# sebproell/4C

Measured on AMD Instinct MI355X. Metric: element-evaluations/sec (hex8 linear elasticity, K+r global assembly), higher is better.
Workload: dtype f64; 1 GPU; hex8-linear-100^3-per-gpu; elements_global=1000000, elements_evaluated_per_gpu=1000000, dofs_owned_rank0=3090903, nnz_rank0=245438109

## Files before the change

4c_amd/csrc/fcg_context.cpp:

```cpp
#include <hip/hip_runtime.h>

#include <algorithm>
#include <chrono>
#include <climits>
#include <cstdlib>
#include <cstring>
#include <mutex>
#include <string>
#include <thread>
#include <vector>

#include "fcg_internal.hpp"
#include "fcg_status.hpp"
#include "fcg_shape.hpp"

namespace {

namespace plan = fcg::create;

std::mutex g_err_mutex;
std::string g_create_error;

void set_create_error(const std::string& s)
{
  std::lock_guard<std::mutex> lk(g_err_mutex);
  g_create_error = s;
}

template <class T>
hipError_t upload(T** dst, const T* src, int64_t n, int64_t& bytes)
{
  *dst = nullptr;
  if (n == 0) return hipSuccess;
  hipError_t e = hipMalloc(reinterpret_cast<void**>(dst), sizeof(T) * n);
  if (e != hipSuccess) return e;
  bytes += sizeof(T) * n;
  if (src) return hipMemcpy(*dst, src, sizeof(T) * n, hipMemcpyHostToDevice);
  return hipSuccess;
}

void free_mesh(fcg::DeviceMesh& m)
{
  void* ptrs[] = {m.node_dof_row, m.node_dof_kcol, m.mass_ptr, m.mass_inc, m.mass_tab, m.mass_rho, m.mass_bad, m.stress_tab, m.stress_bad, m.stress_slot, m.explicit_work, m.ele_mat, m.apply_ye, m.apply_dof, m.diag_de, m.diag_dbc, m.gather_dummy, m.multi_ptr, m.rec_row0, m.rec_meta, m.rec_base, m.rec_ele, m.rec_a, m.rec_tmap, m.ele_orig, m.inc_ele, m.inc_a, m.asm_order, m.ele_x,
      m.ele_dof, m.ele_nodes, m.ele_gid, m.node_x, m.node_dof_col, m.inc_of, m.inc_ptr,
      m.rownode_row0, m.inc_pos, m.rowptr, m.scratch, m.err, m.elem_at, m.lat_x, m.lat_dof,
      m.plane_rec, m.reg_rec, m.reg_tile, m.reg_pos,
      m.tables, m.stamps, m.col_lid, m.diag_pos, m.pcg_work, m.krylov_work, m.col_ele, m.ele_ft, m.inc_row0, m.ele_gp,
      m.pen_ptr, m.ele_nb, m.h27_rows, m.h27_rslot0, m.h27_slot};
  for (void* p : ptrs)
    if (p) (void)hipFree(p);
  if (m.err_host) (void)hipHostFree(m.err_host);
  m = fcg::DeviceMesh{};
}

int graph_on_device(const fcg_desc* d, const int32_t* kcol, std::vector<int64_t>& rowptr,
    std::vector<int32_t>& col, std::string& why)
{
  const int npe = d->celltype == FCG_HEX27 ? 27 : 8;
  if (d->n_rows % 3 != 0)
  {
    why = "n_rows must be 3 x owned nodes";
    return FCG_ERR_ARG;
  }
  for (int64_t n = 0; n < d->n_node; ++n)
    if (kcol[n] < 0 || (d->node_dof_row[n] >= 0 && d->node_dof_row[n] % 3 != 0))
    {
      why = "node DOF LIDs must be non-negative and owned rows start at multiples of 3";
      return FCG_ERR_ARG;
    }
// ... 187 lines not shown
  m.sweep_defer = de && de[0] ? de[0] == '1' : d->kinematics == FCG_LINEAR;
  const char* se = std::getenv("FCG_SWEEP_SKIP_EMPTY");
  m.sweep_skip_empty = !(se && se[0] == '0');
  U.up(&m.elem_at, sp.elem_at);
  U.up(&m.lat_x, sp.lat_x);
  U.up(&m.lat_dof, sp.lat_dof);
  U.up(&m.plane_rec, sp.plane_rec);
  const char* rg = std::getenv("FCG_SWEEP_REGULAR");
  const bool regular = !(rg && rg[0] == '0') && d->kinematics == FCG_LINEAR;
  m.layers_total = sp.layers_total;
  m.reg_layers = regular ? sp.reg_layers : 0;
  if (m.reg_layers > 0)
  {
    U.up(&m.reg_rec, sp.reg_rec);
    U.up(&m.reg_tile, sp.reg_tile);
  }
  else
  {
    const std::vector<uint32_t> no_rec(fcg::REG_REC_WORDS, 0u);
    const std::vector<int32_t> no_run(sp.reg_tile.size(), 0);
    U.up(&m.reg_rec, no_rec);
    U.up(&m.reg_tile, no_run);
  }
  int32_t pos32[32] = {};
  std::copy(sp.reg_pos, sp.reg_pos + 27, pos32);
  U.up(&m.reg_pos, pos32, 32);
  std::vector<double> tab(8 * 8 * 3 * 2 + 8 + 24);
  double xi[81], w[27], xn[81];
  fcg::gauss_rule(fcg::kHex8, xi, w);
  fcg::node_param_coords(fcg::kHex8, xn);
  for (int g = 0; g < 8; ++g) fcg::shape_deriv(fcg::kHex8, &xi[3 * g], &tab[24 * g]);
  for (int g = 0; g < 8; ++g) fcg::shape_deriv(fcg::kHex8, &xn[3 * g], &tab[192 + 24 * g]);
  for (int g = 0; g < 8; ++g) tab[384 + g] = w[g];
  for (int k = 0; k < 24; ++k) tab[392 + k] = xi[k];
  U.up(&m.tables, tab);
  const char* ck = std::getenv("FCG_SWEEP_CHECKED");
  if (U.he == hipSuccess) U.chk(fcg::sweep_geometry_pass(m, ck && ck[0] == '1', U.ctx->stream));
}

void upload_colored(Uploader& U, const fcg_desc* d, const plan::Incidences& I, const plan::ColorHost& cp)
{
  fcg::DeviceMesh& m = U.ctx->mesh;
  m.path = FCG_PATH_COLORED;
  U.up(&m.inc_of, I.inc_of);
  U.up(&m.inc_pos, I.inc_pos);
  U.up(&m.inc_row0, I.inc_row0);
  m.h27_pencil = d->material == FCG_MAT_STVK;
  if (m.h27_pencil)
  {
    fcg::upload_h27_tables();
    U.up(&m.col_ele, cp.pen_ele.data(), d->n_ele);
    U.up(&m.pen_ptr, cp.pen_ptr);
    U.up(&m.ele_nb, cp.nb.data(), d->n_ele);
    for (int c = 0; c < 5; ++c) m.pen_color[c] = cp.pen_color[c];
  }
  else
  {
    U.up(&m.col_ele, cp.col_ele.data(), d->n_ele);
    U.up(&m.ele_ft, cp.ft.data(), d->n_ele);
    for (int c = 0; c < 9; ++c) m.color_ptr[c] = cp.color_ptr[c];
// ... 503 lines not shown
  return FCG_OK;
}

int fcg_get_timing(const fcg_ctx* ctx, double* ms_element, double* ms_assemble)
{
  if (!ctx) return FCG_ERR_ARG;
  read_timing(const_cast<fcg_ctx*>(ctx)->timing);
  if (ms_element) *ms_element = ctx->timing.ms_element;
  if (ms_assemble) *ms_assemble = ctx->timing.ms_assemble;
  return 2;
}

int fcg_get_diagnostics(const fcg_ctx* ctx, uint64_t* out, int n)
{
  if (!ctx || !out || n < 0) return FCG_ERR_ARG;
  const fcg::DeviceMesh& m = ctx->mesh;
  unsigned long long v[16] = {};
  if (m.stamps && hipMemcpy(v, m.stamps, sizeof(v), hipMemcpyDeviceToHost) != hipSuccess)
    return fcg_device_error();
  v[15] = m.path != FCG_PATH_STRUCTURED ? FCG_SWEEP_KERNEL_NA
                                        : (m.sweep_checked ? FCG_SWEEP_KERNEL_CHECKED : FCG_SWEEP_KERNEL_UNCHECKED);
  v[13] = m.path == FCG_PATH_STRUCTURED && !m.sweep_checked ? uint64_t(m.reg_layers) : 0;
  v[14] = m.path == FCG_PATH_STRUCTURED ? uint64_t(m.layers_total) : 0;
  v[12] = m.path != FCG_PATH_STRUCTURED ? FCG_SWEEP_ROWS_NA
                                        : (m.sweep_defer ? FCG_SWEEP_ROWS_DEFERRED : FCG_SWEEP_ROWS_DIRECT);
  for (int i = 0; i < n && i < 16; ++i) out[i] = v[i];
  return m.stamps ? 16 : 0;
}

int fcg_get_create_phases(const fcg_ctx* ctx, double* out, int n)
{
  if (!ctx || (!out && n > 0)) return FCG_ERR_ARG;
  for (int i = 0; i < n && i < 8; ++i) out[i] = ctx->create_phase_s[i];
  return 8;
}

int fcg_get_info(const fcg_ctx* ctx, fcg_info* info)
{
  if (!ctx || !info) return FCG_ERR_ARG;
  const fcg::DeviceMesh& m = ctx->mesh;
  info->n_ele = m.n_ele;
  info->n_node = m.n_node;
  info->n_rows = m.n_rows;
  info->n_cols = m.n_cols;
  info->nnz = m.nnz;
  info->n_incidences = m.n_inc;
// ... 138 lines not shown
```

4c_amd/csrc/fcg_create_plan.cpp:

```cpp
#include "fcg_create_plan.hpp"

#include <array>
#include <climits>
#include <cstdlib>
#include <cstring>
#include <map>
#include <mutex>

#include "fcg_shape.hpp"

namespace fcg {
namespace create {

const int kOff8[8][3] = {{0, 0, 0}, {1, 0, 0}, {1, 1, 0}, {0, 1, 0}, {0, 0, 1}, {1, 0, 1}, {1, 1, 1},
    {0, 1, 1}};

uint64_t morton_key(const double* x, const double* lo, const double* hi)
{
  uint64_t key = 0;
  uint32_t q[3];
  for (int k = 0; k < 3; ++k)
  {
    const double ext = hi[k] - lo[k];
    const double t = ext > 0 ? (x[k] - lo[k]) / ext : 0.0;
// ... 389 lines not shown
  P.tiles_x = (P.n[0] + 3) / 4;
  P.tiles_y = (P.n[1] + 3) / 4;
  const int64_t txy = int64_t(P.tiles_x) * P.tiles_y;
  const char* wenv = std::getenv("FCG_SWEEP_WGS_PER_CU");
  const int wpc = wenv ? std::max(1, std::atoi(wenv)) : 2;
  const char* tenv = std::getenv("FCG_SWEEP_TOTLAG_WGS_PER_CU");
  const int tpc = tenv ? std::max(1, std::atoi(tenv)) : 1;
  const int64_t slots = int64_t(std::max(1, cus)) * (d->kinematics == FCG_TOTLAG ? tpc : wpc);
  int64_t nseg = 1;
  double best = 0.0;
  for (int64_t k = 1; k <= std::min<int64_t>(P.n[2], 64); ++k)
  {
    const int64_t segk = (P.n[2] + k - 1) / k;
    const int64_t wgs = txy * ((P.n[2] + segk - 1) / segk);
    const double cost = double((wgs + slots - 1) / slots) * double(segk + 1);
    if (k == 1 || cost < best)
    {
      best = cost;
      nseg = k;
    }
  }
  P.seg = int32_t((P.n[2] + nseg - 1) / nseg);
  P.tiles_z = (P.n[2] + P.seg - 1) / P.seg;
  P.lat_x.assign(3 * NXn * NYn * NZn, 0.0);
  P.lat_dof.assign(NXn * NYn * NZn, -1);
  for (int64_t nd = 0; nd < d->n_node; ++nd)
  {
    if (npos[nd] < 0) continue;
    for (int k = 0; k < 3; ++k) P.lat_x[3 * npos[nd] + k] = d->node_x[3 * nd + k];
    P.lat_dof[npos[nd]] = d->node_dof_col[nd];
  }
  const int64_t W = fcg::PLANE_REC_WORDS;
  P.plane_rec.assign(int64_t(P.tiles_y) * P.tiles_x * P.n[2] * W, 0u);
  parallel_for(int64_t(P.tiles_y) * P.tiles_x * P.n[2], [&](int64_t idx) {
    const int64_t k = idx % P.n[2];
    const int64_t t = idx / P.n[2];
    const int64_t tx = t % P.tiles_x, ty = t / P.tiles_x;
    uint32_t* rec = P.plane_rec.data() + idx * W;
    uint16_t* np = reinterpret_cast<uint16_t*>(rec + 64);
    for (int c = 0; c < 16; ++c)
    {
      const int64_t i = 4 * tx + c % 4, jj = 4 * ty + c / 4;
      int32_t r = -1;
      if (i < P.n[0] && jj < P.n[1]) r = P.rownode_at[(k * P.n[1] + jj) * P.n[0] + i];
      if (r < 0)
      {
        rec[c] = 0xFFFFFFFFu;
        for (int q = 0; q < 27; ++q) np[27 * c + q] = 0xFFFF;
        continue;
      }
      const int64_t base = d->rowptr[row0[r]];
      rec[c] = uint32_t(row0[r]);
      rec[16 + c] = uint32_t(d->rowptr[row0[r] + 1] - base);
      rec[32 + 2 * c] = uint32_t(uint64_t(base) & 0xFFFFFFFFu);
      rec[32 + 2 * c + 1] = uint32_t(uint64_t(base) >> 32);
      for (int q = 0; q < 27; ++q) np[27 * c + q] = P.nbr_pos[r * 27 + q];
    }
  });
  classify_regular_tiles(P);
  return true;
}

void classify_regular_tiles(StructHost& P)
{
  const int64_t W = fcg::PLANE_REC_WORDS, NK = P.n[2];
  const int64_t ntile = int64_t(P.tiles_y) * P.tiles_x;
  P.reg_rec.assign(ntile * NK * REG_REC_WORDS, 0u);
  P.reg_tile.assign(2 * ntile, 0);
  std::fill(P.reg_pos, P.reg_pos + 27, 0);
  P.reg_layers = 0;
  P.layers_total = 0;
  std::map<std::array<uint16_t, 27>, int64_t> seen;
  const int64_t nrn = int64_t(P.nbr_pos.size()) / 27;
  for (int64_t r = 0; r < nrn; ++r)
  {
    std::array<uint16_t, 27> a;
    bool full = true;
    for (int t = 0; t < 27; ++t)
    {
      a[t] = P.nbr_pos[r * 27 + t];
      full = full && a[t] != 0xFFFF;
    }
// ... 643 lines not shown
```

4c_amd/csrc/fcg_create_plan.hpp:

```cpp
#pragma once

#include <algorithm>
#include <atomic>
#include <cstdint>
#include <string>
#include <thread>
#include <vector>

#include "fourc_gpu.h"

namespace fcg {

constexpr int PLANE_REC_WORDS = 288;
constexpr int REG_REC_WORDS = 16;

namespace create {

template <class F>
void parallel_for(int64_t n, F f)
{
  unsigned nt = std::max(1u, std::min(16u, std::thread::hardware_concurrency()));
  if (n < 4096) nt = 1;
  std::vector<std::thread> th;
  std::atomic<int64_t> next{0};
  const int64_t chunk = 1024;
  auto body = [&]() {
    for (;;)
    {
      const int64_t s = next.fetch_add(chunk);
      if (s >= n) break;
      const int64_t e = std::min(n, s + chunk);
      for (int64_t i = s; i < e; ++i) f(i);
    }
  };
  for (unsigned t = 1; t < nt; ++t) th.emplace_back(body);
  body();
  for (auto& t : th) t.join();
// ... 16 lines not shown
  bool triple_rows = true;
  std::vector<int64_t> diag;
  bool rowcol = false;
  bool square_local = false;
  bool owned_cols_first = false;
  int64_t nrn() const { return int64_t(rownodes.size()); }
};
int build_node_rows(const fcg_desc* d, NodeRows& N, std::string& why);
void build_operator_support(const fcg_desc* d, NodeRows& N);

struct StructHost {
  int32_t lo[3] = {0, 0, 0}, n[3] = {0, 0, 0};
  int32_t elo[3] = {0, 0, 0}, en[3] = {0, 0, 0};
  int32_t tiles_x = 0, tiles_y = 0, tiles_z = 0, seg = 0;
  std::vector<int32_t> elem_at, rownode_at;
  std::vector<uint16_t> nbr_pos;
  std::vector<double> lat_x;
  std::vector<int32_t> lat_dof;
  std::vector<uint32_t> plane_rec;
  std::vector<uint32_t> reg_rec;
  std::vector<int32_t> reg_tile;
  int32_t reg_pos[27] = {};
  int64_t reg_layers = 0, layers_total = 0;
};
void classify_regular_tiles(StructHost& P);
bool detect_lattice_hex8(const fcg_desc* d, std::vector<int32_t>& ijk, std::vector<int32_t>& canon,
    std::string& why);
bool build_structured_plan(const fcg_desc* d, const std::vector<int32_t>& rownodes,
    const std::vector<int32_t>& row0, const int32_t* kcol, int cus, StructHost& P, std::string& why);

struct ColorHost {
  std::vector<int32_t> col_ele;
  std::vector<uint8_t> ft;
  int64_t color_ptr[9] = {0, 0, 0, 0, 0, 0, 0, 0, 0};
  std::vector<int32_t> pen_ele;
  std::vector<int64_t> pen_ptr;
  int64_t pen_color[5] = {0, 0, 0, 0, 0};
  std::vector<uint32_t> nb;
};
bool build_colored_plan(const fcg_desc* d, ColorHost& P, std::string& why);

struct PathChoice {
  bool structured = false, colored = false, gather = false;
  StructHost sp;
  ColorHost cp;
  int path() const
  {
// ... 54 lines not shown
```

4c_amd/csrc/fcg_internal.hpp:

```cpp
#pragma once

#include <hip/hip_runtime.h>

#include <cstdint>
#include <string>
#include <vector>

#include "fcg_create_plan.hpp"
#include "fourc_gpu.h"

namespace fcg {

#ifndef FCG_REC27
#define FCG_REC27 256
#endif
constexpr int64_t record_doubles(int npe) { return npe == 27 ? int64_t(FCG_REC27) : 9 * int64_t(npe) + 3; }

struct DeviceMesh {
  int celltype = 0, kinem = 0, npe = 8;
  int64_t n_ele = 0, n_node = 0, n_rows = 0, n_cols = 0, nnz = 0;
  int64_t n_rownodes = 0, n_inc = 0;
  double lambda = 0, mu = 0, cdiag = 0;
  int material = FCG_MAT_STVK;
  double nh_c = 0, nh_beta = 0;
// ... 49 lines not shown
  int64_t h27_nslab = 0, h27_slab = 0, h27_ring = 0;
  int h27_el_grid = 512;
  std::vector<int64_t> h27_asm_ptr;
  int32_t* h27_rows = nullptr;
  int32_t* h27_rslot0 = nullptr;
  int32_t* h27_slot = nullptr;

  int path = FCG_PATH_GENERAL;
  int32_t tiles_x = 0, tiles_y = 0, tiles_z = 0, seg_planes = 0;
  int32_t I0 = 0, J0 = 0, K0 = 0, NI = 0, NJ = 0, NK = 0;
  int32_t EX0 = 0, EY0 = 0, EZ0 = 0, EX = 0, EY = 0, EZ = 0;
  bool sweep_defer = false;
  bool sweep_skip_empty = true;
  int32_t geom_code = 0, geom_ele = INT32_MAX;
  bool geom_neg = false, sweep_checked = true;
  int32_t* elem_at = nullptr;
  double* lat_x = nullptr;
  int32_t* lat_dof = nullptr;
  uint32_t* plane_rec = nullptr;
  uint32_t* reg_rec = nullptr;
  int32_t* reg_tile = nullptr;
  int32_t* reg_pos = nullptr;
  int64_t reg_layers = 0, layers_total = 0;
  double* tables = nullptr;
  unsigned long long* stamps = nullptr;

  int32_t* col_lid = nullptr;
  int64_t* diag_pos = nullptr;
  bool square_local = false;
  bool owned_cols_first = false;
  bool triple_rows = true;
  double* pcg_work = nullptr;
  int64_t pcg_n = 0;

  int32_t* node_dof_row = nullptr;
  int32_t* node_dof_kcol = nullptr;
  int64_t* mass_ptr = nullptr;
  int64_t* mass_inc = nullptr;
  double* mass_tab = nullptr;
  double* mass_rho = nullptr;
  int32_t* mass_bad = nullptr;

  double* stress_tab = nullptr;
  double* stress_xinv = nullptr;
  int32_t* stress_bad = nullptr;
  int32_t* stress_slot = nullptr;
// ... 106 lines not shown
```

4c_amd/csrc/fcg_sweep.hip:

```cpp
#include <hip/hip_runtime.h>

#include <type_traits>

#include "fcg_hex8_element.hpp"
#include "fcg_internal.hpp"
#include "fcg_visit_table.h"

namespace fcg {

namespace {

constexpr int TX = 4, TY = 4;
constexpr int EXN = TX + 1, EYN = TY + 1;
constexpr int NSLOT = EXN * EYN;
constexpr int NXN = TX + 2;
constexpr int NNODE = NXN * (TY + 2);
constexpr int PR_ROW0 = 0, PR_LEN = 16, PR_BASE = 32, PR_NPOS = 64;
__device__ constexpr int nx_sw(int p, int slot) { return (p + 4 * (slot & 1)) & 7; }
__device__ constexpr int nx2i(int d, int p, int slot, int n)
{
  return (((d * 4 + p) * NSLOT + slot) * 8 + (n ^ nx_sw(p, slot))) * 2;
}

__device__ constexpr int node_ox(int n) { return ((n & 3) == 1 || (n & 3) == 2) ? 1 : 0; }
// ... 3 lines not shown
struct SweepArgs {
  const double* u_col;
  const double* lat_x;
  const int32_t* lat_dof;
  const int32_t* elem_at;
  const uint32_t* plane_rec;
  const uint32_t* reg_rec;
  const int32_t* reg_tile;
  const int32_t* reg_pos;
  const double* tables;
  double* K;
  double* fint;
  int32_t* err;
  unsigned long long* stamps;
  StVK mat;
  const double* v_col;
  const double* T_col;
  const double* Ngp;
  double* Kst;
  double* Kts;
  double* Ktt;
  double* fT;
  double tsi_m, tsi_T0, tsi_k, tsi_kts;
  int32_t tiles_x, tiles_y, seg_planes;
  int32_t I0, J0, K0, NI, NJ, NK;
  int32_t EX0, EY0, EZ0, EX, EY, EZ;
  int32_t skip_empty;
};

template <bool TSI>
constexpr int node_comps() { return TSI ? 10 : 6; }

#ifndef FCG_GP_STRIDE
#define FCG_GP_STRIDE 18
#endif
#ifndef FCG_TG_STRIDE
#define FCG_TG_STRIDE 4
#endif

template <int KIN, bool TSI, bool TH = false, bool DEFER = false>
struct SweepShared {
  alignas(16) double nx[3 * 4 * NSLOT * 8 * 2];
  alignas(16) double gp[KIN ? 8 : 1][KIN ? NSLOT : 1][KIN ? FCG_GP_STRIDE : 16];
  alignas(16) double tg[TSI ? 8 : 1][TSI ? NSLOT : 1][TSI ? FCG_TG_STRIDE : 4];
  double node[3][NNODE][node_comps<TSI>()];
  uint32_t prec[3][PLANE_REC_WORDS];
  double gxi[8][4];
  double Ng[TSI ? 8 : 1][8];
  alignas(16) double NgT[TSI ? 8 : 1][10];
  double w8[8];
// ... 393 lines not shown
  if (A.stamps && tid == 0)                                                                        \
  {                                                                                                \
    const unsigned long long now = __builtin_amdgcn_s_memtime();                                  \
    st_acc[i] += now - st_last;                                                                    \
    st_last = now;                                                                                 \
  }

template <int KIN, bool WANT_K, bool OVERWRITE, int MODE, bool CHECKED = true>
#ifndef FCG_SWEEP_WGS
#define FCG_SWEEP_WGS 2
#endif
__global__ __launch_bounds__(256, KIN ? 1 : FCG_SWEEP_WGS) void sweep_h8_kernel(SweepArgs A)
{
  constexpr bool TSI = MODE == 1 || MODE == 2, TH = MODE == 2, DEFER = MODE == 3, GEOM = MODE == 4;
  static_assert(!GEOM || (KIN == 0 && !WANT_K && CHECKED), "the geometry pass is one instantiation");
  static_assert(CHECKED || !TSI, "the TSI passes keep the checks");
  static_assert(!TSI || (KIN == 0 && WANT_K), "TSI is geometrically linear, full tangent");
  static_assert(!DEFER || WANT_K, "deferred blocks are K blocks");
  __shared__ SweepShared<KIN, TSI, TH, DEFER> sh;
  constexpr int NACC = TH ? 8 : ((KIN || TSI) ? 16 : 9);
  constexpr int NC = node_comps<TSI>();
  constexpr int NLD = (NNODE * NC + 255) / 256;
  constexpr int NF = TSI ? 4 : 3;
  const int tid = threadIdx.x;
  unsigned long long st_acc[3] = {0, 0, 0};
  unsigned long long st_last = A.stamps ? __builtin_amdgcn_s_memtime() : 0ull;
  const int tile = blockIdx.x;
  const int tx = tile % A.tiles_x;
  const int ty = (tile / A.tiles_x) % A.tiles_y;
  const int tz = tile / (A.tiles_x * A.tiles_y);
  const int i0 = A.I0 + TX * tx, j0 = A.J0 + TY * ty;
  const int kz0 = A.K0 + A.seg_planes * tz;
  const int kz1 = min(kz0 + A.seg_planes, A.K0 + A.NK);
  const uint32_t* prec_tile = A.plane_rec + (int64_t(ty) * A.tiles_x + tx) * A.NK * PLANE_REC_WORDS;
  const int64_t LX = A.EX + 1, LY = A.EY + 1;
  constexpr bool REGK = (MODE == 0 || MODE == 3) && KIN == 0 && !CHECKED;
  int rlo = 0, rhi = 0;
  const uint32_t* creg_tile = nullptr;
  if constexpr (REGK)
  {
    const int64_t txy = int64_t(ty) * A.tiles_x + tx;
    rlo = max(A.K0 + A.reg_tile[2 * txy], kz0);
    rhi = min(A.K0 + A.reg_tile[2 * txy + 1], kz1) - 1;
    creg_tile = A.reg_rec + txy * A.NK * REG_REC_WORDS;
  }
  auto reg_layer = [&](int L) -> bool { return REGK && L >= rlo && L < rhi; };
  auto reg_plane = [&](int p) -> bool { return REGK && p > rlo && p < rhi; };

  if (tid < 24) sh.gxi[tid / 3][tid % 3] = A.tables[392 + tid];
  if (tid < 8) sh.w8[tid] = A.tables[384 + tid];
  if (TSI && tid < 64)
  {
    (&sh.Ng[0][0])[tid] = A.Ngp[tid];
    sh.NgT[TSI ? (tid & 7) : 0][tid >> 3] = A.Ngp[tid];
  }

  const int s = tid >> 3, g = tid & 7;
  const bool a_lane = s < NSLOT;
  const int sx = s % EXN, sy = s / EXN;
  const int ex = i0 - 1 + sx, ey = j0 - 1 + sy;
  const bool exy_in = a_lane && ex >= A.EX0 && ex < A.EX0 + A.EX && ey >= A.EY0 && ey < A.EY0 + A.EY;
  auto load_elem = [&](int lz) -> int {
    if (reg_layer(lz)) return a_lane ? 0 : -1;
    if (!exy_in || lz < A.EZ0 || lz >= A.EZ0 + A.EZ) return -1;
    return A.elem_at[(int64_t(lz - A.EZ0) * A.EY + (ey - A.EY0)) * A.EX + (ex - A.EX0)];
  };
  bool n_lane[NLD], nxy_in[NLD];
  int ncol[NLD], ncomp[NLD];
  int64_t nlat_xy[NLD];
#pragma unroll
  for (int j = 0; j < NLD; ++j)
  {
    const int v = tid + 256 * j;
    n_lane[j] = v < NNODE * NC;
    ncol[j] = v / NC;
    ncomp[j] = v - NC * (v / NC);
    const int ni = i0 - 1 + ncol[j] % NXN, nj = j0 - 1 + ncol[j] / NXN;
    nxy_in[j] = n_lane[j] && ni >= A.EX0 && ni <= A.EX0 + A.EX && nj >= A.EY0 && nj <= A.EY0 + A.EY;
    nlat_xy[j] = nxy_in[j] ? int64_t(nj - A.EY0) * LX + (ni - A.EX0) : 0;
  }
  auto node_li = [&](int j, int P) -> int64_t { return int64_t(P - A.EZ0) * LX * LY + nlat_xy[j]; };
  auto node_in = [&](int j, int P) -> bool { return nxy_in[j] && P >= A.EZ0 && P <= A.EZ0 + A.EZ; };
  auto load_dof = [&](int j, int P) -> int32_t {
    if (GEOM || !node_in(j, P) || ncomp[j] < 3) return -1;
    return A.lat_dof[node_li(j, P)];
  };
  auto load_val = [&](int j, int P, int32_t dof) -> double {
    const int cp = ncomp[j];
    const bool has = node_in(j, P) && (cp < 3 || dof >= 0);
    const double* src = A.lat_x + (3 * node_li(j, P) + cp);
    if (cp >= 3) src = A.u_col + (dof + cp - 3);
    if (TSI && cp >= 6) src = A.v_col + (dof + cp - 6);
    if (TSI && cp >= 9) src = A.T_col + dof / 3;
    return has ? *src : 0.0;
  };
  auto load_node = [&](int j, int P) -> double { return load_val(j, P, load_dof(j, P)); };
  auto load_rec = [&](int p, uint32_t* w) {
    const bool in = p >= kz0 && p < kz1;
    const uint32_t* src = prec_tile + int64_t(in ? p - A.K0 : 0) * PLANE_REC_WORDS;
    const bool cp = reg_plane(p);
    if (cp) src = creg_tile + int64_t(p - A.K0) * REG_REC_WORDS;
#pragma unroll
    for (int k = 0; k < 2; ++k)
    {
      const int v = tid + 256 * k;
      if (v < PLANE_REC_WORDS) w[k] = (in && (!cp || v < 12)) ? src[v] : (v < PR_LEN ? 0xFFFFFFFFu : 0u);
    }
  };
  auto store_rec = [&](int p, const uint32_t* w) {
    const bool cp = reg_plane(p);
#pragma unroll
    for (int k = 0; k < 2; ++k)
    {
      const int v = tid + 256 * k;
      const int at = cp ? (v < 4 ? PR_ROW0 + 4 * v : PR_BASE + 8 * (((v - 4) >> 1) & 3) + (v & 1)) : v;
      if (v < PLANE_REC_WORDS && (!cp || v < 12)) sh.prec[ring(p)][at] = w[k];
    }
  };

  const int c = tid >> 4, k = tid & 15;
  const int cx = c % TX, cy = c / TX;
  const uint32_t vis0 = kVisit[k][0], vis1 = kVisit[k][1];
  int32_t rp_a = 0, rp_b = 0, rp_s = 0;
  if constexpr (REGK && WANT_K)
  {
    rp_a = A.reg_pos[(vis0 >> 16) & 31] + 243 * cx;
    rp_b = A.reg_pos[(vis1 >> 16) & 31] + 243 * cx;
    rp_s = A.reg_pos[(vis1 >> 11) & 31] + 243 * cx;
  }

  constexpr bool SKIPE = KIN == 0 && !TSI && !GEOM;
  const bool skip_e = SKIPE && A.skip_empty != 0;
  const int L0 = (skip_e && kz0 - 1 < A.EZ0) ? kz0 : kz0 - 1;
#pragma unroll
  for (int j = 0; j < NLD; ++j)
    if (n_lane[j])
    {
      sh.node[ring(L0)][ncol[j]][ncomp[j]] = load_node(j, L0);
      sh.node[ring(L0 + 1)][ncol[j]][ncomp[j]] = load_node(j, L0 + 1);
    }
  {
    uint32_t w[2];
    load_rec(L0, w);
    store_rec(L0, w);
    load_rec(L0 + 1, w);
    store_rec(L0 + 1, w);
  }
  int32_t dof_nxt[NLD];
#pragma unroll
  for (int j = 0; j < NLD; ++j) dof_nxt[j] = n_lane[j] ? load_dof(j, L0 + 2) : -1;
  int e_cur = load_elem(L0);
  for (int v = tid; v < int(sizeof(sh.hold) / sizeof(double)); v += 256) (&sh.hold[0][0][0])[v] = 0.0;
  if constexpr (DEFER)
// ... 462 lines not shown
#ifdef FCG_PROBE_TH_NORMW
            if (OVERWRITE)
#else
            if (OVERWRITE && !TH)
#endif
              A.fint[row0 + d] = fp[d] + f[d];
            else
              A.fint[row0 + d] += fp[d] + f[d];
          }
          if (TSI)
          {
            if (OVERWRITE)
              A.fT[row0 / 3] = fp[NF - 1] + f[NF - 1];
            else
              A.fT[row0 / 3] += fp[NF - 1] + f[NF - 1];
          }
        }
      }
    }
    e_cur = e_nxt;
    __syncthreads();
    FCG_STAMP(1);
  }
  if (A.stamps && tid == 0)
  {
    for (int i = 0; i < 3; ++i) atomicAdd(&A.stamps[i], st_acc[i]);
    atomicAdd(&A.stamps[5], 1ull);
  }
}

}

namespace {
SweepArgs sweep_args(const DeviceMesh& m, const double* d_u_col, double* d_K, double* d_fint)
{
  SweepArgs a{};
  a.u_col = d_u_col;
  a.lat_x = m.lat_x;
  a.lat_dof = m.lat_dof;
  a.elem_at = m.elem_at;
  a.plane_rec = m.plane_rec;
  a.reg_rec = m.reg_rec;
  a.reg_tile = m.reg_tile;
  a.reg_pos = m.reg_pos;
  a.tables = m.tables;
  a.K = d_K;
  a.fint = d_fint;
  a.err = m.err;
  a.stamps = m.stamps;
  a.mat = StVK{m.lambda, m.mu, m.cdiag};
  a.tiles_x = m.tiles_x;
  a.tiles_y = m.tiles_y;
  a.seg_planes = m.seg_planes;
  a.I0 = m.I0; a.J0 = m.J0; a.K0 = m.K0; a.NI = m.NI; a.NJ = m.NJ; a.NK = m.NK;
  a.EX0 = m.EX0; a.EY0 = m.EY0; a.EZ0 = m.EZ0; a.EX = m.EX; a.EY = m.EY; a.EZ = m.EZ;
  a.skip_empty = m.sweep_skip_empty ? 1 : 0;
  return a;
}
}

#define FCG_SWEEP_C(KIN, CHECKED)                                                                  \
  if (want_k && m.sweep_defer && overwrite)                                                        \
    hipLaunchKernelGGL((sweep_h8_kernel<KIN, true, true, 3, CHECKED>), grid, block, 0, stream, a);  \
  else if (want_k && m.sweep_defer)                                                                \
    hipLaunchKernelGGL((sweep_h8_kernel<KIN, true, false, 3, CHECKED>), grid, block, 0, stream, a); \
  else if (want_k && overwrite)                                                                    \
    hipLaunchKernelGGL((sweep_h8_kernel<KIN, true, true, 0, CHECKED>), grid, block, 0, stream, a);  \
  else if (want_k)                                                                                 \
    hipLaunchKernelGGL((sweep_h8_kernel<KIN, true, false, 0, CHECKED>), grid, block, 0, stream, a); \
  else if (overwrite)                                                                              \
    hipLaunchKernelGGL((sweep_h8_kernel<KIN, false, true, 0, CHECKED>), grid, block, 0, stream, a); \
  else                                                                                             \
    hipLaunchKernelGGL((sweep_h8_kernel<KIN, false, false, 0, CHECKED>), grid, block, 0, stream, a);
#define FCG_SWEEP(KIN)                                                                             \
  if (m.sweep_checked)                                                                             \
  {                                                                                                \
    FCG_SWEEP_C(KIN, true)                                                                         \
  }                                                                                                \
  else                                                                                             \
  {                                                                                                \
    FCG_SWEEP_C(KIN, false)                                                                        \
  }

hipError_t launch_sweep_h8_totlag(const DeviceMesh& m, const double* d_u_col, bool want_k,
    bool overwrite, double* d_K, double* d_fint, hipStream_t stream);

#ifdef FCG_SWEEP_TOTLAG_TU
hipError_t launch_sweep_h8_totlag(const DeviceMesh& m, const double* d_u_col, bool want_k,
    bool overwrite, double* d_K, double* d_fint, hipStream_t stream)
{
  const int64_t ntiles = int64_t(m.tiles_x) * m.tiles_y * m.tiles_z;
  if (ntiles == 0) return hipSuccess;
  const SweepArgs a = sweep_args(m, d_u_col, d_K, d_fint);
  const dim3 grid{static_cast<unsigned>(ntiles), 1, 1};
  const dim3 block{256, 1, 1};
  FCG_SWEEP(1)
  return hipGetLastError();
}
#else
hipError_t launch_sweep_h8(const DeviceMesh& m, const double* d_u_col, bool want_k,
    bool overwrite, double* d_K, double* d_fint, hipStream_t stream)
{
  if (m.kinem != 0) return launch_sweep_h8_totlag(m, d_u_col, want_k, overwrite, d_K, d_fint, stream);
  const int64_t ntiles = int64_t(m.tiles_x) * m.tiles_y * m.tiles_z;
  if (ntiles == 0) return hipSuccess;
  const SweepArgs a = sweep_args(m, d_u_col, d_K, d_fint);
  const dim3 grid{static_cast<unsigned>(ntiles), 1, 1};
  const dim3 block{256, 1, 1};
  FCG_SWEEP(0)
  return hipGetLastError();
}

hipError_t sweep_geometry_pass(DeviceMesh& m, bool force_checked, hipStream_t stream)
{
  m.geom_code = 0;
  m.geom_ele = INT32_MAX;
  m.geom_neg = false;
  m.sweep_checked = true;
  const int64_t ntiles = int64_t(m.tiles_x) * m.tiles_y * m.tiles_z;
  if (ntiles > 0)
  {
    int32_t* d_out = nullptr;
    int32_t out[3] = {0, INT32_MAX, 0};
    hipError_t he = hipMalloc(reinterpret_cast<void**>(&d_out), sizeof(out));
    if (he != hipSuccess) return he;
    he = hipMemcpyAsync(d_out, out, sizeof(out), hipMemcpyHostToDevice, stream);
    if (he == hipSuccess)
    {
      SweepArgs a = sweep_args(m, nullptr, nullptr, nullptr);
      a.err = d_out;
      a.stamps = nullptr;
      const dim3 grid{static_cast<unsigned>(ntiles), 1, 1};
      const dim3 block{256, 1, 1};
      hipLaunchKernelGGL((sweep_h8_kernel<0, false, false, 4>), grid, block, 0, stream, a);
      he = hipGetLastError();
    }
    if (he == hipSuccess) he = hipMemcpyAsync(out, d_out, sizeof(out), hipMemcpyDeviceToHost, stream);
    if (he == hipSuccess) he = hipStreamSynchronize(stream);
    (void)hipFree(d_out);
    if (he != hipSuccess) return he;
    m.geom_code = out[0];
    m.geom_ele = out[1];
    m.geom_neg = out[2] != 0;
  }
  m.sweep_checked = force_checked || m.geom_code != 0 || m.geom_neg;
  return hipSuccess;
}

hipError_t launch_sweep_h8_tsi(const DeviceMesh& m, const double* d_u_col, bool overwrite,
    double* d_K, double* d_fint, const SweepTsi& t, hipStream_t stream)
{
  const int64_t ntiles = int64_t(m.tiles_x) * m.tiles_y * m.tiles_z;
  if (ntiles == 0) return hipSuccess;
  SweepArgs a = sweep_args(m, d_u_col, d_K, d_fint);
  a.v_col = t.v_col;
  a.T_col = t.T_col;
  a.Ngp = t.Ngp;
  a.Kst = t.Kst;
  a.Kts = t.Kts;
  a.Ktt = t.Ktt;
  a.fT = t.fT;
  a.tsi_m = t.m;
  a.tsi_T0 = t.T0;
  a.tsi_k = t.conduct;
  a.tsi_kts = t.kts;
  const dim3 grid{static_cast<unsigned>(ntiles), 1, 1};
  const dim3 block{256, 1, 1};
  if (!t.split)
  {
    if (overwrite)
      hipLaunchKernelGGL((sweep_h8_kernel<0, true, true, 1>), grid, block, 0, stream, a);
    else
      hipLaunchKernelGGL((sweep_h8_kernel<0, true, false, 1>), grid, block, 0, stream, a);
    return hipGetLastError();
  }
  if (overwrite)
  {
    hipLaunchKernelGGL((sweep_h8_kernel<0, true, true, 0>), grid, block, 0, stream, a);
    hipLaunchKernelGGL((sweep_h8_kernel<0, true, true, 2>), grid, block, 0, stream, a);
  }
  else
  {
    hipLaunchKernelGGL((sweep_h8_kernel<0, true, false, 0>), grid, block, 0, stream, a);
    hipLaunchKernelGGL((sweep_h8_kernel<0, true, false, 2>), grid, block, 0, stream, a);
  }
  return hipGetLastError();
}
#endif
#undef FCG_SWEEP
// ... 4 lines not shown
```

4c_amd/fcg.py:

```python

import ctypes
import os

import numpy as np

PKG_DIR = os.path.dirname(os.path.abspath(__file__))
LIB_PATH = os.path.join(PKG_DIR, "lib", "libfourc_gpu.so")
if os.environ.get("FCG_LIB"):
    LIB_PATH = os.path.join(PKG_DIR, "lib", "libfourc_gpu_%s.so" % os.environ["FCG_LIB"])

HEX8, HEX27 = 0, 1
LINEAR, TOTLAG = 0, 1
CALC_NLNSTIFF, CALC_INTERNALFORCE = 0, 1
ACCUMULATE, OVERWRITE = 0, 1
PATH_AUTO, PATH_GENERAL, PATH_STRUCTURED, PATH_COLORED, PATH_GATHER = 0, 1, 2, 3, 4
MAT_STVK, MAT_ELASTHYPER_COUPNEOHOOKE = 0, 1
TSI_STRUCT_FORCE, TSI_STIFFTEMP, TSI_THERMO_FINTCOND, TSI_COUPLTANG = 1, 2, 4, 8
TSI_ALL = 15
STRESS_NONE, STRESS_PK2, STRESS_CAUCHY = 0, 1, 2
STRAIN_NONE, STRAIN_GL, STRAIN_EA = 0, 1, 2
ABI_VERSION = 2

FCG_OK, FCG_ERR_NODAL_DETJ, FCG_ERR_SINGULAR, FCG_ERR_ARG, FCG_ERR_DEVICE = 0, 1, 2, 3, 4
STATUS = {0: "FCG_OK", 1: "FCG_ERR_NODAL_DETJ", 2: "FCG_ERR_SINGULAR", 3: "FCG_ERR_ARG",
# ... 926 lines not shown
        buf = (ctypes.c_uint64 * 16)()
        n = lib().fcg_get_diagnostics(self._h, buf, 16)
        return list(buf) if n > 0 else None

    SWEEP_KERNELS = ("not applicable", "checked", "unchecked")

    def sweep_kernel(self):
        buf = (ctypes.c_uint64 * 16)()
        lib().fcg_get_diagnostics(self._h, buf, 16)
        return self.SWEEP_KERNELS[int(buf[15])]

    SWEEP_ROWS = ("not applicable", "direct", "deferred")

    def sweep_rows(self):
        buf = (ctypes.c_uint64 * 16)()
        lib().fcg_get_diagnostics(self._h, buf, 16)
        return self.SWEEP_ROWS[int(buf[12])]

    def sweep_regular_layers(self):
        buf = (ctypes.c_uint64 * 16)()
        lib().fcg_get_diagnostics(self._h, buf, 16)
        return int(buf[13]), int(buf[14])

    CREATE_PHASES = ("checks", "graph_device", "node_rows", "lattice_plans", "incidences",
                     "incidence_positions", "device_plans", "total")

    def create_phases(self):
        buf = (ctypes.c_double * 8)()
        lib().fcg_get_create_phases(self._h, buf, 8)
        return dict(zip(self.CREATE_PHASES, list(buf)))

    def timing(self):
        a, b = ctypes.c_double(), ctypes.c_double()
        lib().fcg_get_timing(self._h, ctypes.byref(a), ctypes.byref(b))
        return a.value, b.value


def gmres_options(restart=None, max_iter=None, rtol=None, precond=None):
    opt = FcgGmresOptions()
    lib().fcg_gmres_default_options(ctypes.byref(opt))
    for k, v in (("restart", restart), ("max_iter", max_iter), ("precond", precond)):
        if v is not None:
            setattr(opt, k, int(v))
    if rtol is not None:
        opt.rtol = float(rtol)
    return opt
# ... 230 lines not shown
```

Measured before the change: 1.188 billion element-evaluations/s.

## Drive sweep kernel from per-block chain records of tile z-segments

Replaces the fixed tile-by-z-segment grid mapping with a host-built table of chains. Each chain lists up to four (tile, kz0, kz1) pieces, and each block loops over the pieces in its record. The default chains match the previous segmentation, so default behaviour should be equivalent. Env vars FCG_SWEEP_CHAINS can select balanced multi-piece or stacked chains, meant to cut tail imbalance and the repeated warm-up plane per segment. The per-block constant setup moves out of the piece loop, and the kernel gains a loop with kernarg re-reads, which may raise register pressure.

```diff
diff --git a/4c_amd/csrc/fcg_context.cpp b/4c_amd/csrc/fcg_context.cpp
--- a/4c_amd/csrc/fcg_context.cpp
+++ b/4c_amd/csrc/fcg_context.cpp
@@ -44,7 +44,7 @@
   void* ptrs[] = {m.node_dof_row, m.node_dof_kcol, m.mass_ptr, m.mass_inc, m.mass_tab, m.mass_rho, m.mass_bad, m.stress_tab, m.stress_bad, m.stress_slot, m.explicit_work, m.ele_mat, m.apply_ye, m.apply_dof, m.diag_de, m.diag_dbc, m.gather_dummy, m.multi_ptr, m.rec_row0, m.rec_meta, m.rec_base, m.rec_ele, m.rec_a, m.rec_tmap, m.ele_orig, m.inc_ele, m.inc_a, m.asm_order, m.ele_x,
       m.ele_dof, m.ele_nodes, m.ele_gid, m.node_x, m.node_dof_col, m.inc_of, m.inc_ptr,
       m.rownode_row0, m.inc_pos, m.rowptr, m.scratch, m.err, m.elem_at, m.lat_x, m.lat_dof,
-      m.plane_rec, m.reg_rec, m.reg_tile, m.reg_pos,
+      m.plane_rec, m.reg_rec, m.reg_tile, m.reg_pos, m.chains, m.seg_chains == m.chains ? nullptr : m.seg_chains,
       m.tables, m.stamps, m.col_lid, m.diag_pos, m.pcg_work, m.krylov_work, m.col_ele, m.ele_ft, m.inc_row0, m.ele_gp,
       m.pen_ptr, m.ele_nb, m.h27_rows, m.h27_rslot0, m.h27_slot};
   for (void* p : ptrs)
@@ -278,6 +278,15 @@
     U.up(&m.reg_rec, no_rec);
     U.up(&m.reg_tile, no_run);
   }
+  U.up(&m.chains, sp.chains.rec);
+  m.n_chains = sp.chains.n;
+  m.chain_longest = sp.chains.longest;
+  m.chain_shortest = sp.chains.shortest;
+  if (sp.chains.rec == sp.seg_chains.rec)
+    m.seg_chains = m.chains;
+  else
+    U.up(&m.seg_chains, sp.seg_chains.rec);
+  m.n_seg_chains = sp.seg_chains.n;
   int32_t pos32[32] = {};
   std::copy(sp.reg_pos, sp.reg_pos + 27, pos32);
   U.up(&m.reg_pos, pos32, 32);
@@ -292,6 +301,14 @@
   U.up(&m.tables, tab);
   const char* ck = std::getenv("FCG_SWEEP_CHECKED");
   if (U.he == hipSuccess) U.chk(fcg::sweep_geometry_pass(m, ck && ck[0] == '1', U.ctx->stream));
+  if (m.sweep_checked && m.chains != m.seg_chains)
+  {
+    (void)hipFree(m.chains);
+    m.chains = m.seg_chains;
+    m.n_chains = sp.seg_chains.n;
+    m.chain_longest = sp.seg_chains.longest;
+    m.chain_shortest = sp.seg_chains.shortest;
+  }
 }
 
 void upload_colored(Uploader& U, const fcg_desc* d, const plan::Incidences& I, const plan::ColorHost& cp)
@@ -841,6 +858,12 @@
                                         : (m.sweep_checked ? FCG_SWEEP_KERNEL_CHECKED : FCG_SWEEP_KERNEL_UNCHECKED);
   v[13] = m.path == FCG_PATH_STRUCTURED && !m.sweep_checked ? uint64_t(m.reg_layers) : 0;
   v[14] = m.path == FCG_PATH_STRUCTURED ? uint64_t(m.layers_total) : 0;
+  if (m.path == FCG_PATH_STRUCTURED)
+  {
+    v[9] = uint64_t(m.n_chains);
+    v[10] = uint64_t(m.chain_longest);
+    v[11] = uint64_t(m.chain_shortest);
+  }
   v[12] = m.path != FCG_PATH_STRUCTURED ? FCG_SWEEP_ROWS_NA
                                         : (m.sweep_defer ? FCG_SWEEP_ROWS_DEFERRED : FCG_SWEEP_ROWS_DIRECT);
   for (int i = 0; i < n && i < 16; ++i) out[i] = v[i];
diff --git a/4c_amd/csrc/fcg_create_plan.cpp b/4c_amd/csrc/fcg_create_plan.cpp
--- a/4c_amd/csrc/fcg_create_plan.cpp
+++ b/4c_amd/csrc/fcg_create_plan.cpp
@@ -435,6 +435,18 @@
   }
   P.seg = int32_t((P.n[2] + nseg - 1) / nseg);
   P.tiles_z = (P.n[2] + P.seg - 1) / P.seg;
+  const char* senv = std::getenv("FCG_SWEEP_SKIP_EMPTY");
+  P.skip_bottom = d->kinematics == FCG_LINEAR && !(senv && senv[0] == '0') && P.lo[2] - 1 < P.elo[2];
+  build_sweep_chains(P, 0, P.seg_chains);
+  P.chains = P.seg_chains;
+  const char* cenv = std::getenv("FCG_SWEEP_CHAINS");
+  if (d->kinematics == FCG_LINEAR)
+  {
+    if (cenv && cenv[0] == 's')
+      build_stacked_chains(P, std::max(1, std::atoi(cenv + 1)), P.chains);
+    else if (cenv && cenv[0])
+      build_sweep_chains(P, std::max(0, std::atoi(cenv)), P.chains);
+  }
   P.lat_x.assign(3 * NXn * NYn * NZn, 0.0);
   P.lat_dof.assign(NXn * NYn * NZn, -1);
   for (int64_t nd = 0; nd < d->n_node; ++nd)
@@ -471,6 +483,128 @@
     }
   });
   classify_regular_tiles(P);
+  return true;
+}
+
+void build_sweep_chains(const StructHost& P, int64_t want, StructHost::Chains& C)
+{
+  const int64_t NK = P.n[2], T = int64_t(P.tiles_x) * P.tiles_y;
+  C = StructHost::Chains{};
+  if (NK <= 0 || T <= 0) return;
+  auto warm = [&](int64_t k) -> int64_t { return (k == 0 && P.skip_bottom) ? 0 : 1; };
+  std::vector<int32_t> cost;
+  auto finish = [&]() {
+    C.n = int32_t(cost.size());
+    C.longest = *std::max_element(cost.begin(), cost.end());
+    C.shortest = *std::min_element(cost.begin(), cost.end());
+  };
+  if (want <= 0)
+  {
+    for (int64_t tz = 0; tz < P.tiles_z; ++tz)
+      for (int64_t t = 0; t < T; ++t)
+      {
+        const int64_t kz0 = int64_t(P.seg) * tz, kz1 = std::min<int64_t>(kz0 + P.seg, NK);
+        int32_t r[SWEEP_CHAIN_WORDS] = {int32_t(t), int32_t(kz0), int32_t(kz1), 0};
+        C.rec.insert(C.rec.end(), r, r + SWEEP_CHAIN_WORDS);
+        cost.push_back(int32_t(kz1 - kz0 + warm(kz0)));
+      }
+    finish();
+    return;
+  }
+  int64_t n = std::min<int64_t>(want, T * NK);
+  for (;;)
+  {
+    C.rec.clear();
+    cost.clear();
+    int64_t t = 0, k = 0;
+    bool capped = false;
+    while (t < T)
+    {
+      const int64_t m = std::max<int64_t>(1, n - int64_t(cost.size()));
+      const int64_t left = (T - t) * NK - k + warm(k) + (T - t - 1) * warm(0) + (m - 1);
+      const int64_t target = std::max<int64_t>((left + m - 1) / m, warm(k) + 1);
+      int32_t r[SWEEP_CHAIN_WORDS] = {};
+      int64_t c = 0;
+      int np = 0;
+      while (t < T && np < SWEEP_CHAIN_PIECES && target - c > warm(k))
+      {
+        const int64_t take = std::min(NK - k, target - c - warm(k));
+        r[4 * np] = int32_t(t);
+        r[4 * np + 1] = int32_t(k);
+        r[4 * np + 2] = int32_t(k + take);
+        c += take + warm(k);
+        ++np;
+        k += take;
+        if (k == NK)
+        {
+          k = 0;
+          ++t;
+        }
+      }
+      capped = capped || (t < T && target - c > warm(k));
+      C.rec.insert(C.rec.end(), r, r + SWEEP_CHAIN_WORDS);
+      cost.push_back(int32_t(c));
+    }
+    if (!capped) break;
+    n = std::max<int64_t>(n + 1, int64_t(cost.size()));
+  }
+  finish();
+}
+
+bool build_stacked_chains(const StructHost& P, int64_t slots, StructHost::Chains& C)
+{
+  const int64_t NK = P.n[2], T = int64_t(P.tiles_x) * P.tiles_y;
+  C = P.seg_chains;
+  if (NK <= 0 || T <= 0 || slots <= 0) return false;
+  const int64_t q = T / slots, R = T % slots;
+  int64_t seg2 = NK, tz2 = 1, rounds2 = R > 0 ? 1 : 0;
+  if (R > 0)
+  {
+    double best = 0.0;
+    for (int64_t k = 1; k <= std::min<int64_t>(NK, 64); ++k)
+    {
+      const int64_t segk = (NK + k - 1) / k, tzk = (NK + segk - 1) / segk;
+      const int64_t rounds = (R * tzk + slots - 1) / slots;
+      const double cost = double(rounds) * double(segk + 1);
+      if (k == 1 || cost < best)
+      {
+        best = cost;
+        seg2 = segk;
+        tz2 = tzk;
+        rounds2 = rounds;
+      }
+    }
+  }
+  if (q == 0 || q + rounds2 > SWEEP_CHAIN_PIECES) return false;
+  auto warm = [&](int64_t k) -> int64_t { return (k == 0 && P.skip_bottom) ? 0 : 1; };
+  C = StructHost::Chains{};
+  std::vector<int32_t> cost;
+  for (int64_t j = 0; j < slots; ++j)
+  {
+    int32_t r[SWEEP_CHAIN_WORDS] = {};
+    int np = 0;
+    int64_t c = 0;
+    auto piece = [&](int64_t t, int64_t k0, int64_t k1) {
+      r[4 * np] = int32_t(t);
+      r[4 * np + 1] = int32_t(k0);
+      r[4 * np + 2] = int32_t(k1);
+      c += k1 - k0 + warm(k0);
+      ++np;
+    };
+    for (int64_t w = 0; w < q; ++w) piece(w * slots + j, 0, NK);
+    for (int64_t w = 0; w < rounds2; ++w)
+    {
+      const int64_t p = w * slots + j;
+      if (p >= R * tz2) break;
+      const int64_t tz = p / R;
+      piece(q * slots + p % R, tz * seg2, std::min((tz + 1) * seg2, NK));
+    }
+    C.rec.insert(C.rec.end(), r, r + SWEEP_CHAIN_WORDS);
+    cost.push_back(int32_t(c));
+  }
+  C.n = int32_t(cost.size());
+  C.longest = *std::max_element(cost.begin(), cost.end());
+  C.shortest = *std::min_element(cost.begin(), cost.end());
   return true;
 }
 
diff --git a/4c_amd/csrc/fcg_create_plan.hpp b/4c_amd/csrc/fcg_create_plan.hpp
--- a/4c_amd/csrc/fcg_create_plan.hpp
+++ b/4c_amd/csrc/fcg_create_plan.hpp
@@ -13,6 +13,8 @@
 
 constexpr int PLANE_REC_WORDS = 288;
 constexpr int REG_REC_WORDS = 16;
+constexpr int SWEEP_CHAIN_PIECES = 4;
+constexpr int SWEEP_CHAIN_WORDS = 4 * SWEEP_CHAIN_PIECES;
 
 namespace create {
 
@@ -75,7 +77,15 @@
   std::vector<int32_t> reg_tile;
   int32_t reg_pos[27] = {};
   int64_t reg_layers = 0, layers_total = 0;
+  struct Chains {
+    std::vector<int32_t> rec;
+    int32_t n = 0, longest = 0, shortest = 0;
+  };
+  Chains chains, seg_chains;
+  bool skip_bottom = false;
 };
+void build_sweep_chains(const StructHost& P, int64_t want, StructHost::Chains& C);
+bool build_stacked_chains(const StructHost& P, int64_t slots, StructHost::Chains& C);
 void classify_regular_tiles(StructHost& P);
 bool detect_lattice_hex8(const fcg_desc* d, std::vector<int32_t>& ijk, std::vector<int32_t>& canon,
     std::string& why);
diff --git a/4c_amd/csrc/fcg_internal.hpp b/4c_amd/csrc/fcg_internal.hpp
--- a/4c_amd/csrc/fcg_internal.hpp
+++ b/4c_amd/csrc/fcg_internal.hpp
@@ -95,6 +95,9 @@
   int32_t* reg_tile = nullptr;
   int32_t* reg_pos = nullptr;
   int64_t reg_layers = 0, layers_total = 0;
+  int32_t* chains = nullptr;
+  int32_t* seg_chains = nullptr;
+  int32_t n_chains = 0, n_seg_chains = 0, chain_longest = 0, chain_shortest = 0;
   double* tables = nullptr;
   unsigned long long* stamps = nullptr;
 
diff --git a/4c_amd/csrc/fcg_sweep.hip b/4c_amd/csrc/fcg_sweep.hip
--- a/4c_amd/csrc/fcg_sweep.hip
+++ b/4c_amd/csrc/fcg_sweep.hip
@@ -49,10 +49,11 @@
   double* Ktt;
   double* fT;
   double tsi_m, tsi_T0, tsi_k, tsi_kts;
-  int32_t tiles_x, tiles_y, seg_planes;
+  int32_t tiles_x, tiles_y;
   int32_t I0, J0, K0, NI, NJ, NK;
   int32_t EX0, EY0, EZ0, EX, EY, EZ;
   int32_t skip_empty;
+  const int32_t* chains;
 };
 
 template <bool TSI>
@@ -492,44 +493,68 @@
   constexpr int NC = node_comps<TSI>();
   constexpr int NLD = (NNODE * NC + 255) / 256;
   constexpr int NF = TSI ? 4 : 3;
-  const int tid = threadIdx.x;
+  const int tid0 = threadIdx.x;
   unsigned long long st_acc[3] = {0, 0, 0};
   unsigned long long st_last = A.stamps ? __builtin_amdgcn_s_memtime() : 0ull;
-  const int tile = blockIdx.x;
-  const int tx = tile % A.tiles_x;
-  const int ty = (tile / A.tiles_x) % A.tiles_y;
-  const int tz = tile / (A.tiles_x * A.tiles_y);
-  const int i0 = A.I0 + TX * tx, j0 = A.J0 + TY * ty;
-  const int kz0 = A.K0 + A.seg_planes * tz;
-  const int kz1 = min(kz0 + A.seg_planes, A.K0 + A.NK);
-  const uint32_t* prec_tile = A.plane_rec + (int64_t(ty) * A.tiles_x + tx) * A.NK * PLANE_REC_WORDS;
   const int64_t LX = A.EX + 1, LY = A.EY + 1;
+  if (tid0 < 24) sh.gxi[tid0 / 3][tid0 % 3] = A.tables[392 + tid0];
+  if (tid0 < 8) sh.w8[tid0] = A.tables[384 + tid0];
+  if (TSI && tid0 < 64)
+  {
+    (&sh.Ng[0][0])[tid0] = A.Ngp[tid0];
+    sh.NgT[TSI ? (tid0 & 7) : 0][tid0 >> 3] = A.Ngp[tid0];
+  }
   constexpr bool REGK = (MODE == 0 || MODE == 3) && KIN == 0 && !CHECKED;
+  const int c = tid0 >> 4, k = tid0 & 15;
+  const int cx = c % TX, cy = c / TX;
+  const uint32_t vis0 = kVisit[k][0], vis1 = kVisit[k][1];
+  int32_t rp_a = 0, rp_b = 0, rp_s = 0;
+  if constexpr (REGK && WANT_K)
+  {
+    rp_a = A.reg_pos[(vis0 >> 16) & 31] + 243 * cx;
+    rp_b = A.reg_pos[(vis1 >> 16) & 31] + 243 * cx;
+    rp_s = A.reg_pos[(vis1 >> 11) & 31] + 243 * cx;
+  }
+
+  constexpr int kPieces = (KIN == 0 && !TSI && !GEOM && !CHECKED) ? SWEEP_CHAIN_PIECES : 1;
+  typedef const SweepArgs __attribute__((address_space(4)))* ArgSegment;
+  ArgSegment Ap = (ArgSegment)__builtin_amdgcn_kernarg_segment_ptr();
+#pragma nounroll
+  for (int piece = 0; piece < kPieces; ++piece)
+  {
+  if constexpr (kPieces > 1) __asm__ volatile("" : "+s"(Ap));
+  int tid_piece = tid0;
+  if constexpr (kPieces > 1) __asm__ volatile("" : "+v"(tid_piece));
+  const int tid = tid_piece;
+#define FCG_COLD(f) (kPieces > 1 ? Ap->f : A.f)
+  const int32_t* chain = FCG_COLD(chains) + (int64_t(blockIdx.x) * SWEEP_CHAIN_WORDS + 4 * piece);
+  const int tile = __builtin_amdgcn_readfirstlane(chain[0]);
+  const int kz0 = FCG_COLD(K0) + __builtin_amdgcn_readfirstlane(chain[1]);
+  const int kz1 = FCG_COLD(K0) + __builtin_amdgcn_readfirstlane(chain[2]);
+  if (kz0 >= kz1) break;
+  const int tx = tile % FCG_COLD(tiles_x);
+  const int ty = tile / FCG_COLD(tiles_x);
+  const int i0 = FCG_COLD(I0) + TX * tx, j0 = FCG_COLD(J0) + TY * ty;
+  const uint32_t* prec_tile = FCG_COLD(plane_rec) + int64_t(tile) * FCG_COLD(NK) * PLANE_REC_WORDS;
+  const int cEX0 = FCG_COLD(EX0), cEY0 = FCG_COLD(EY0), cEX = FCG_COLD(EX), cEY = FCG_COLD(EY);
   int rlo = 0, rhi = 0;
   const uint32_t* creg_tile = nullptr;
   if constexpr (REGK)
   {
-    const int64_t txy = int64_t(ty) * A.tiles_x + tx;
-    rlo = max(A.K0 + A.reg_tile[2 * txy], kz0);
-    rhi = min(A.K0 + A.reg_tile[2 * txy + 1], kz1) - 1;
-    creg_tile = A.reg_rec + txy * A.NK * REG_REC_WORDS;
+    const int32_t* run = FCG_COLD(reg_tile) + 2 * tile;
+    rlo = max(FCG_COLD(K0) + __builtin_amdgcn_readfirstlane(run[0]), kz0);
+    rhi = min(FCG_COLD(K0) + __builtin_amdgcn_readfirstlane(run[1]), kz1) - 1;
+    creg_tile = FCG_COLD(reg_rec) + int64_t(tile) * FCG_COLD(NK) * REG_REC_WORDS;
+#undef FCG_COLD
   }
   auto reg_layer = [&](int L) -> bool { return REGK && L >= rlo && L < rhi; };
   auto reg_plane = [&](int p) -> bool { return REGK && p > rlo && p < rhi; };
-
-  if (tid < 24) sh.gxi[tid / 3][tid % 3] = A.tables[392 + tid];
-  if (tid < 8) sh.w8[tid] = A.tables[384 + tid];
-  if (TSI && tid < 64)
-  {
-    (&sh.Ng[0][0])[tid] = A.Ngp[tid];
-    sh.NgT[TSI ? (tid & 7) : 0][tid >> 3] = A.Ngp[tid];
-  }
 
   const int s = tid >> 3, g = tid & 7;
   const bool a_lane = s < NSLOT;
   const int sx = s % EXN, sy = s / EXN;
   const int ex = i0 - 1 + sx, ey = j0 - 1 + sy;
-  const bool exy_in = a_lane && ex >= A.EX0 && ex < A.EX0 + A.EX && ey >= A.EY0 && ey < A.EY0 + A.EY;
+  const bool exy_in = a_lane && ex >= cEX0 && ex < cEX0 + cEX && ey >= cEY0 && ey < cEY0 + cEY;
   auto load_elem = [&](int lz) -> int {
     if (reg_layer(lz)) return a_lane ? 0 : -1;
     if (!exy_in || lz < A.EZ0 || lz >= A.EZ0 + A.EZ) return -1;
@@ -546,8 +571,8 @@
     ncol[j] = v / NC;
     ncomp[j] = v - NC * (v / NC);
     const int ni = i0 - 1 + ncol[j] % NXN, nj = j0 - 1 + ncol[j] / NXN;
-    nxy_in[j] = n_lane[j] && ni >= A.EX0 && ni <= A.EX0 + A.EX && nj >= A.EY0 && nj <= A.EY0 + A.EY;
-    nlat_xy[j] = nxy_in[j] ? int64_t(nj - A.EY0) * LX + (ni - A.EX0) : 0;
+    nxy_in[j] = n_lane[j] && ni >= cEX0 && ni <= cEX0 + cEX && nj >= cEY0 && nj <= cEY0 + cEY;
+    nlat_xy[j] = nxy_in[j] ? int64_t(nj - cEY0) * (int64_t(cEX) + 1) + (ni - cEX0) : 0;
   }
   auto node_li = [&](int j, int P) -> int64_t { return int64_t(P - A.EZ0) * LX * LY + nlat_xy[j]; };
   auto node_in = [&](int j, int P) -> bool { return nxy_in[j] && P >= A.EZ0 && P <= A.EZ0 + A.EZ; };
@@ -588,17 +613,6 @@
     }
   };
 
-  const int c = tid >> 4, k = tid & 15;
-  const int cx = c % TX, cy = c / TX;
-  const uint32_t vis0 = kVisit[k][0], vis1 = kVisit[k][1];
-  int32_t rp_a = 0, rp_b = 0, rp_s = 0;
-  if constexpr (REGK && WANT_K)
-  {
-    rp_a = A.reg_pos[(vis0 >> 16) & 31] + 243 * cx;
-    rp_b = A.reg_pos[(vis1 >> 16) & 31] + 243 * cx;
-    rp_s = A.reg_pos[(vis1 >> 11) & 31] + 243 * cx;
-  }
-
   constexpr bool SKIPE = KIN == 0 && !TSI && !GEOM;
   const bool skip_e = SKIPE && A.skip_empty != 0;
   const int L0 = (skip_e && kz0 - 1 < A.EZ0) ? kz0 : kz0 - 1;
@@ -1107,7 +1121,8 @@
     __syncthreads();
     FCG_STAMP(1);
   }
-  if (A.stamps && tid == 0)
+  }
+  if (A.stamps && tid0 == 0)
   {
     for (int i = 0; i < 3; ++i) atomicAdd(&A.stamps[i], st_acc[i]);
     atomicAdd(&A.stamps[5], 1ull);
@@ -1136,7 +1151,7 @@
   a.mat = StVK{m.lambda, m.mu, m.cdiag};
   a.tiles_x = m.tiles_x;
   a.tiles_y = m.tiles_y;
-  a.seg_planes = m.seg_planes;
+  a.chains = m.chains;
   a.I0 = m.I0; a.J0 = m.J0; a.K0 = m.K0; a.NI = m.NI; a.NJ = m.NJ; a.NK = m.NK;
   a.EX0 = m.EX0; a.EY0 = m.EY0; a.EZ0 = m.EZ0; a.EX = m.EX; a.EY = m.EY; a.EZ = m.EZ;
   a.skip_empty = m.sweep_skip_empty ? 1 : 0;
@@ -1174,10 +1189,9 @@
 hipError_t launch_sweep_h8_totlag(const DeviceMesh& m, const double* d_u_col, bool want_k,
     bool overwrite, double* d_K, double* d_fint, hipStream_t stream)
 {
-  const int64_t ntiles = int64_t(m.tiles_x) * m.tiles_y * m.tiles_z;
-  if (ntiles == 0) return hipSuccess;
+  if (m.n_chains == 0) return hipSuccess;
   const SweepArgs a = sweep_args(m, d_u_col, d_K, d_fint);
-  const dim3 grid{static_cast<unsigned>(ntiles), 1, 1};
+  const dim3 grid{static_cast<unsigned>(m.n_chains), 1, 1};
   const dim3 block{256, 1, 1};
   FCG_SWEEP(1)
   return hipGetLastError();
@@ -1187,10 +1201,9 @@
     bool overwrite, double* d_K, double* d_fint, hipStream_t stream)
 {
   if (m.kinem != 0) return launch_sweep_h8_totlag(m, d_u_col, want_k, overwrite, d_K, d_fint, stream);
-  const int64_t ntiles = int64_t(m.tiles_x) * m.tiles_y * m.tiles_z;
-  if (ntiles == 0) return hipSuccess;
+  if (m.n_chains == 0) return hipSuccess;
   const SweepArgs a = sweep_args(m, d_u_col, d_K, d_fint);
-  const dim3 grid{static_cast<unsigned>(ntiles), 1, 1};
+  const dim3 grid{static_cast<unsigned>(m.n_chains), 1, 1};
   const dim3 block{256, 1, 1};
   FCG_SWEEP(0)
   return hipGetLastError();
@@ -1202,8 +1215,7 @@
   m.geom_ele = INT32_MAX;
   m.geom_neg = false;
   m.sweep_checked = true;
-  const int64_t ntiles = int64_t(m.tiles_x) * m.tiles_y * m.tiles_z;
-  if (ntiles > 0)
+  if (m.n_seg_chains > 0)
   {
     int32_t* d_out = nullptr;
     int32_t out[3] = {0, INT32_MAX, 0};
@@ -1215,7 +1227,8 @@
       SweepArgs a = sweep_args(m, nullptr, nullptr, nullptr);
       a.err = d_out;
       a.stamps = nullptr;
-      const dim3 grid{static_cast<unsigned>(ntiles), 1, 1};
+      a.chains = m.seg_chains;
+      const dim3 grid{static_cast<unsigned>(m.n_seg_chains), 1, 1};
       const dim3 block{256, 1, 1};
       hipLaunchKernelGGL((sweep_h8_kernel<0, false, false, 4>), grid, block, 0, stream, a);
       he = hipGetLastError();
@@ -1235,9 +1248,9 @@
 hipError_t launch_sweep_h8_tsi(const DeviceMesh& m, const double* d_u_col, bool overwrite,
     double* d_K, double* d_fint, const SweepTsi& t, hipStream_t stream)
 {
-  const int64_t ntiles = int64_t(m.tiles_x) * m.tiles_y * m.tiles_z;
-  if (ntiles == 0) return hipSuccess;
+  if (m.n_seg_chains == 0) return hipSuccess;
   SweepArgs a = sweep_args(m, d_u_col, d_K, d_fint);
+  a.chains = m.seg_chains;
   a.v_col = t.v_col;
   a.T_col = t.T_col;
   a.Ngp = t.Ngp;
@@ -1249,7 +1262,7 @@
   a.tsi_T0 = t.T0;
   a.tsi_k = t.conduct;
   a.tsi_kts = t.kts;
-  const dim3 grid{static_cast<unsigned>(ntiles), 1, 1};
+  const dim3 grid{static_cast<unsigned>(m.n_seg_chains), 1, 1};
   const dim3 block{256, 1, 1};
   if (!t.split)
   {
diff --git a/4c_amd/fcg.py b/4c_amd/fcg.py
--- a/4c_amd/fcg.py
+++ b/4c_amd/fcg.py
@@ -972,6 +972,11 @@
         lib().fcg_get_diagnostics(self._h, buf, 16)
         return int(buf[13]), int(buf[14])
 
+    def sweep_chains(self):
+        buf = (ctypes.c_uint64 * 16)()
+        lib().fcg_get_diagnostics(self._h, buf, 16)
+        return int(buf[9]), int(buf[10]), int(buf[11])
+
     CREATE_PHASES = ("checks", "graph_device", "node_rows", "lattice_plans", "incidences",
                      "incidence_positions", "device_plans", "total")
 
```

Result: no change. 1.187 billion element-evaluations/s (-0.1%).
